# sbelharbi/sr-caco-2

Measured on AMD Instinct MI355X. Metric: train patches/sec, SwinIR x8 64->512 1ch, higher is better.
Workload: dtype f32 (fp16x2 split-MFMA, f32 accumulate)

## Files before the change

include/srhip.h:

```cpp
#ifndef SRHIP_H
#define SRHIP_H
#ifdef __cplusplus
extern "C" {
#endif
#if defined(__GNUC__) || defined(__clang__)
#pragma GCC visibility push(default)
#endif

const char* srhip_last_error(void);
int srhip_abi_version(void);
int srhip_experiments_enabled(void);
int srhip_set_matmul_mode(int mode);
int srhip_get_matmul_mode(void);


int srhip_gemm_nt(const float* A, long lda, const float* W, long ldw, const float* bias, float* C,
                  long ldc, int M, int N, int K, int a_mode, const float* ln_stats, int epi,
                  const float* R, long ldr, const float* rowscale, int rows_per_scale, float alpha,
                  float* aux, long ldaux, void* stream);

int srhip_gemm_nt_batched(const float* A, long lda, long a_z0, long a_z1, const float* W, long ldw, long w_z0, long w_z1, float* C,
                          long ldc, long c_z0, long c_z1, int M, int N, int K, int zcount, int zdiv, void* stream);

int srhip_conv3x3_nhwc(const float* X, long ldx, const float* Wp, const float* bias, float* Y, long ldy,
// ... 134 lines not shown
int srhip_tn_plan_bx3(int M, int NI, int NJ, int conv, int* S, long* part_floats);
int srhip_tn_group_plan_bx3(int M, int ntiles, int* S);
int srhip_gemm_tn_bx3(const float* A, long lda, const float* B, long ldb, int M, int NI, int NJ,
                      const float* a_rowscale, int a_rowscale_rows, int b_mode, const float* ln_stats,
                      float* part, float* part_colsum, int S, void* stream);
int srhip_gemm_tn_grouped_bx3(const srhip_tn_problem* probs, int nprob, int M, int S, void* stream);
int srhip_conv3x3_wgrad_bx3(const float* dY, long lddy, const float* X, long ldx, int B, int H, int W,
                            int Cout, int Cin, float* part, float* part_colsum, int S, void* stream);
int srhip_reduce_linear_wgrad(const float* part, const float* colsum, int S, float* dW, float* db,
                              int N, int K, void* stream);
long srhip_ln_affine_ws(int N, int K);
int srhip_reduce_ln_linear_wgrad(const float* part, const float* colsum, int S, const float* W,
                                 const float* gamma, const float* beta, float* dW, float* db,
                                 float* dgamma, float* dbeta, int N, int K, float* ln_ws,
                                 void* stream);
typedef struct {
  const float* part; const float* colsum;
  const float* W; const float* gamma; const float* beta;
  float* dW; float* db; float* dgamma; float* dbeta;
  int N, K;
  float* ln_ws;
} srhip_reduce_problem;
int srhip_reduce_wgrad_grouped(const srhip_reduce_problem* probs, int nprob, int S, void* stream);
int srhip_reduce_conv_wgrad(const float* part, const float* colsum, int S, float* dW, float* db,
                            int Co, int Ci, void* stream);

int srhip_fold_layernorm(const float* W, const float* b, const float* gamma, const float* beta,
                         float* Wf, float* bf, int N, int K, void* stream);
int srhip_transpose(const float* in, float* out, int R, int C, void* stream);
int srhip_pack_conv_weight(const float* w, float* wp, float* wpt, int Co, int Ci, void* stream);

int srhip_layernorm_fwd(const float* x, float* stats, float* y, const float* gamma, const float* beta,
                        long M, int C, void* stream);
long srhip_layernorm_bwd_ws(long M, int C);
int srhip_layernorm_bwd(const float* dy, const float* x, const float* stats, const float* res,
                        const float* gamma, float* out, float* dgamma, float* dbeta, float* workspace, long M,
                        int C, void* stream);

int srhip_resize_cubic(const void* src, void* dst, int is_u8, int B, int H, int W, int Ho, int Wo, void* stream);
int srhip_u8_to_unit(const unsigned char* src, float* dst, long n, void* stream);
int srhip_clip01(float* x, long n, void* stream);

int srhip_imresize_aa(const void* src, int is_u8, float* tmp, float* dst, int B, int H, int W, int Ho, int Wo, double scale,
                      void* stream);
int srhip_imresize_aa_u16(const unsigned short* src, int in_max, float* tmp, float* dst, int B, int H, int W, int Ho, int Wo,
                          double scale, void* stream);
// ... 293 lines not shown
```

sr-caco-2_amd/csrc/api.hip:

```cpp
#include <stdarg.h>
#include "common.h"
#include "kernels.h"
#include "../../include/srhip.h"

static thread_local char g_err[512] = "";

int sr_fail(int code, const char* fmt, ...) {
  va_list ap;
  va_start(ap, fmt);
  vsnprintf(g_err, sizeof(g_err), fmt, ap);
  va_end(ap);
  return code;
}

extern "C" {

const char* srhip_last_error(void) { return g_err; }
int srhip_abi_version(void) { return 14; }
int srhip_experiments_enabled(void) {
#ifdef SRHIP_EXPERIMENTS
  return 1;
#else
  return 0;
#endif
// ... 423 lines not shown
  SR_REQUIRE(nprob >= 1 && nprob <= (bx ? 24 : 4), "gemm_tn_grouped: 1..%d problems", bx ? 24 : 4);
  SR_REQUIRE(M > 0 && S > 0, "gemm_tn_grouped: empty problem");
  TnArgs a[24];
  memset(a, 0, sizeof(a));
  for (int k = 0; k < nprob; ++k) {
    const srhip_tn_problem& q = probs[k];
    SR_REQUIRE(q.b_mode >= 0 && q.b_mode <= 2, "gemm_tn_grouped: b_mode %d", q.b_mode);
    SR_REQUIRE(q.b_mode != 1 || q.ln_stats, "gemm_tn_grouped: layernorm prologue without stats");
    SR_REQUIRE(!q.a_rowscale || q.a_rowscale_rows > 0, "gemm_tn_grouped: a_rowscale_rows must be > 0");
    TnArgs& p = a[k];
    p.A = q.A; p.lda = q.lda; p.B = q.B; p.ldb = q.ldb; p.M = M; p.NI = q.NI; p.NJ = q.NJ;
    p.a_rowscale = q.a_rowscale; p.a_rowscale_rows = q.a_rowscale_rows; p.b_mode = q.b_mode;
    p.ln_stats = q.ln_stats; p.part = q.part; p.part_colsum = q.part_colsum; p.S = S;
  }
  return bx ? sr_gemm_tnb_grouped(a, nprob, (hipStream_t)stream) : sr_gemm_tn_grouped(a, nprob, (hipStream_t)stream);
}
int srhip_gemm_tn_grouped(const srhip_tn_problem* probs, int nprob, int M, int S, void* stream) {
  return gemm_tn_grouped_any(false, probs, nprob, M, S, stream);
}
int srhip_gemm_tn_grouped_bx3(const srhip_tn_problem* probs, int nprob, int M, int S, void* stream) {
  return gemm_tn_grouped_any(true, probs, nprob, M, S, stream);
}

static int conv3x3_ps2_split(int wfmt, const float* X, long ldx, const void* Wb, const float* bias, float* Yup, long ldy,
                          int B, int H, int W, int Cin, int Cout, int epi, float alpha, void* stream) {
  SR_REQUIRE(epi == 0 || epi == 1 || epi == 6, "conv3x3_ps2_bx3: epi %d (0 bias | 1 relu | 6 leaky relu)", epi);
  NtArgs p;
  memset(&p, 0, sizeof(p));
  p.A = X; p.lda = ldx; p.Wb = (const unsigned short*)Wb; p.C = Yup; p.ldc = ldy;
  p.N = Cout; p.K = Cin; p.bias = bias; p.epi = epi; p.rows_per_scale = H * W; p.alpha = alpha;
  p.batch = B; p.H = H; p.Wd = W; p.ps = 1; p.wfmt = wfmt;
  return sr_conv3x3_ntb(p, (hipStream_t)stream);
}
static int conv3x3_ps2_bwd_data_split(int wfmt, const float* dYup, long lddy, const void* Wbt, float* dX, long ldx, int B, int H,
                                   int W, int Cout, int Cin, int epi, const float* R, long ldr, float alpha,
                                   void* stream) {
  SR_REQUIRE(epi == 0 || ((epi == 4 || epi == 7) && R), "conv3x3_ps2_bwd_data_bx3: epi %d (0 | 4, 7 with R)", epi);
  NtArgs p;
  memset(&p, 0, sizeof(p));
  p.A = dYup; p.lda = lddy; p.Wb = (const unsigned short*)Wbt; p.C = dX; p.ldc = ldx;
  p.N = Cin; p.K = Cout; p.rows_per_scale = H * W; p.alpha = epi == 7 ? alpha : 1.f; p.batch = B; p.H = H; p.Wd = W; p.ps = 2;
  p.epi = epi; p.R = R; p.ldr = ldr; p.wfmt = wfmt;
  return sr_conv3x3_ntb(p, (hipStream_t)stream);
}
int srhip_conv3x3_ps2_bx3(const float* X, long ldx, const void* Wb, const float* bias, float* Yup, long ldy,
                          int B, int H, int W, int Cin, int Cout, int epi, float alpha, void* stream) {
// ... 46 lines not shown
```

sr-caco-2_amd/csrc/gemm_tnb.hip:

```cpp
#include <stdlib.h>
#include "common.h"
#include "kernels.h"

typedef __bf16 bf16x8 __attribute__((ext_vector_type(8)));
typedef __bf16 bf16x2 __attribute__((ext_vector_type(2)));
typedef float f32x2 __attribute__((ext_vector_type(2)));
typedef unsigned u32x4 __attribute__((ext_vector_type(4)));

namespace {

constexpr int TKB = 32;

__device__ const float k_tnb_zero_row[256] = {0.f};

__device__ __forceinline__ f32x16 mfma_bf(u32x4 a, u32x4 b, f32x16 c) {
  return __builtin_amdgcn_mfma_f32_32x32x16_bf16(__builtin_bit_cast(bf16x8, a),
                                                 __builtin_bit_cast(bf16x8, b), c, 0, 0, 0);
}

typedef _Float16 f16x8 __attribute__((ext_vector_type(8)));
typedef _Float16 tn_f16x2 __attribute__((ext_vector_type(2)));
__device__ __forceinline__ f32x16 mfma_h(u32x4 a, u32x4 b, f32x16 c) {
  return __builtin_amdgcn_mfma_f32_32x32x16_f16(__builtin_bit_cast(f16x8, a), __builtin_bit_cast(f16x8, b), c, 0, 0, 0);
}
// ... 307 lines not shown
        const int row = (wi * W + i) * 32 + mfma_row(q, lane);
        if (row < ivalid) {
          const int io = i0 + row;
          out[(long)(p.ps ? (io % ps_f) * 4 + io / ps_f : io) * p.NJ + j0 + col] = acc[i][j][q];
        }
      }
    }
  }

  if (do_colsum) {
    float* red = (float*)smem;
    if (producer && !isB) {
#pragma unroll
      for (int j = 0; j < W; ++j) red[hh * BC + W * lane + j] = cs[j];
    }
    __syncthreads();
    if (tid < ivalid) {
      const int io = i0 + tid;
      p.part_colsum[(long)s * p.NI + (p.ps ? (io % ps_f) * 4 + io / ps_f : io)] = red[tid] + red[BC + tid];
    }
  }
}

template <int W, int BM = -1, bool AR = false, bool NR = false, bool CONV = false>
__device__ __forceinline__ void tnb_body_h(const TnArgs& p, const int s, const int tile, unsigned char* smem, const int tap = 0) {
  const int bmode = BM >= 0 ? BM : p.b_mode;
  const bool arow = BM >= 0 ? AR : (p.a_rowscale != nullptr);
  constexpr int BC = 64 * W, HC = 32 * W;
  constexpr int PLANE = 2 * BC * 64;
  constexpr int BUF = 3 * PLANE;
  constexpr int CTRL = 2 * PLANE;
  constexpr int SINV = 2 * PLANE + 4096;

  const int tid = threadIdx.x, lane = tid & 63;
  const int wave8 = __builtin_amdgcn_readfirstlane(tid >> 6);
  const bool producer = wave8 >= 4;
  const int wave = wave8 & 3;
  const int wi = wave >> 1, wj = wave & 1, r = lane & 31, h = lane >> 5;
  const int nbj = (p.NJ + p.j_tile - 1) / p.j_tile;
  const int bi = tile / nbj, bj = tile - bi * nbj;
  const int i0 = bi * p.i_tile, j0 = bj * p.j_tile;
  const int ivalid = min(p.i_tile, p.NI - i0), jvalid = min(p.j_tile, p.NJ - j0);
  const int m_begin = s * p.rows_per_slice;
  const int m_end = min(p.M, m_begin + p.rows_per_slice);
  const bool do_colsum = p.part_colsum && bj == 0 && tap == 0;
  const int cdy = CONV ? tap / 3 - 1 : 0, cdx = CONV ? tap % 3 - 1 : 0;

  struct Stage {
    typename ColVec<W>::T rv[2][8];
    float scale;
    float2 stats;
    int trow;
  };
  Stage sg0, sg1;
  const bool isB = wave & 1;
  const int ch = wave >> 1;
  const int lt = lane & 31, th = lane >> 5;
  const int opvalid = isB ? jvalid : ivalid;
  const int gcol = HC * ch + W * lt;
  const int colq = max(min(gcol, opvalid - W), 0);
  const int dsh = gcol - colq;
  const bool ragged = NR ? false : opvalid % W != 0;
  const float* const opP = isB ? p.B + j0 : p.A + i0;
  const long opLd = isB ? p.ldb : p.lda;
  const unsigned colb = (unsigned)((16L * th * opLd + colq) * 4);
  float cs[W], sc[W];
#pragma unroll
  for (int j = 0; j < W; ++j) { cs[j] = 0.f; sc[j] = 0x1p126f; }
// ... 256 lines not shown
#pragma unroll
      for (int ks = 0; ks < 2; ++ks) {
        u32x4 fa[W][2];
#pragma unroll
        for (int i = 0; i < W; ++i)
#pragma unroll
          for (int pl = 0; pl < 2; ++pl) fa[i][pl] = *(const u32x4*)(cur + pl * PLANE + a_off[i][ks]);
#pragma unroll
        for (int j = 0; j < W; ++j) {
          const u32x4 bh = *(const u32x4*)(cur + b_off[j][ks]);
          const u32x4 bl = *(const u32x4*)(cur + PLANE + b_off[j][ks]);
#pragma unroll
          for (int i = 0; i < W; ++i) acc[i][j] = mfma_h(fa[i][1], bh, acc[i][j]);
#pragma unroll
          for (int i = 0; i < W; ++i) acc[i][j] = mfma_h(fa[i][0], bl, acc[i][j]);
#pragma unroll
          for (int i = 0; i < W; ++i) acc[i][j] = mfma_h(fa[i][0], bh, acc[i][j]);
        }
      }
      __syncthreads();
    }
    __syncthreads();
    const float* sinv = (const float*)(smem + SINV);
    float* out = p.part + ((long)(s * (CONV ? 9 : 1) + tap) * p.NI) * p.NJ;
#pragma unroll
    for (int i = 0; i < W; ++i)
#pragma unroll
      for (int j = 0; j < W; ++j) {
        const int col = (wj * W + j) * 32 + r;
        if (col >= jvalid) continue;
        const float ib = sinv[BC + col];
#pragma unroll
        for (int q = 0; q < 16; ++q) {
          const int row = (wi * W + i) * 32 + mfma_row(q, lane);
          if (row < ivalid) out[(long)(i0 + row) * p.NJ + j0 + col] = acc[i][j][q] * (sinv[row] * ib);
        }
      }
  }

  if (do_colsum) {
    float* red = (float*)smem;
    if (producer && !isB) {
#pragma unroll
      for (int j = 0; j < W; ++j) red[th * BC + gcol + j] = cs[j];
    }
    __syncthreads();
    if (tid < ivalid) p.part_colsum[(long)s * p.NI + i0 + tid] = red[tid] + red[BC + tid];
  }
}

constexpr int TK9 = 16;
__device__ __forceinline__ int unit_slot9(int col, int u) { return 2 * col + (u ^ ((col >> 3) & 1)); }
constexpr int T9_OPS = 6;
constexpr int T9_PLANE = T9_OPS * 64 * 32;
constexpr int T9_CTRL = 2 * T9_PLANE;
constexpr int T9_BUF = 2 * T9_PLANE + 2048;
constexpr int T9_SINV = 2 * T9_BUF;
constexpr int T9_LDS = 2 * T9_BUF + 2048;
constexpr int T9_THREADS = 14 * 64;

template <int H2, int DBG = 0>
__device__ __forceinline__ void tnb9_consume(const TnArgs& p, const int s, const int i0, const int j0, const int nch,
                                             unsigned char* smem, const int wi, const int wj, const int lane) {
  constexpr int NU = H2 ? 4 : 5;
  constexpr int DY0 = H2 ? 1 : 0;
  const int r = lane & 31, h = lane >> 5;
  f32x16 acc[NU];
#pragma unroll
  for (int u = 0; u < NU; ++u)
#pragma unroll
    for (int q = 0; q < 16; ++q) acc[u][q] = 0.f;
// ... 538 lines not shown
#pragma unroll
  for (int i = 1; i < TNB_GROUP_MAX; ++i)
    if (i < g.n && t >= g.tile_start[i]) { p = g.p[i]; t0 = g.tile_start[i]; }
  tnb_body<W>(p, slice, t - t0, 0, smem);
}

template <int W>
__global__ void __launch_bounds__(512, 1) k_tnb_grouped_h(TnbGroup g) {
  extern __shared__ __attribute__((aligned(16))) unsigned char smem[];
  int slice, t;
  tnb_group_block(g, slice, t);
  TnArgs p = g.p[0];
  int t0 = 0;
#pragma unroll
  for (int i = 1; i < TNB_GROUP_MAX; ++i)
    if (i < g.n && t >= g.tile_start[i]) { p = g.p[i]; t0 = g.tile_start[i]; }
  const bool even = p.NI % W == 0 && p.NJ % W == 0 && p.i_tile % W == 0 && p.j_tile % W == 0;
  if (even && p.b_mode == 1 && !p.a_rowscale) tnb_body_h<W, 1, false, true>(p, slice, t - t0, smem);
  else if (even && p.b_mode == 0 && p.a_rowscale) tnb_body_h<W, 0, true, true>(p, slice, t - t0, smem);
  else if (even && p.b_mode == 2 && p.a_rowscale) tnb_body_h<W, 2, true, true>(p, slice, t - t0, smem);
  else tnb_body_h<W>(p, slice, t - t0, smem);
}

constexpr int TNB_BATCH_MAX = 40;
struct TnbConvBatch {
  TnArgs base;
  const float* A[TNB_BATCH_MAX];
  const float* B[TNB_BATCH_MAX];
  long part_stride, colsum_stride;
  int n, tiles, xcd;
};
template <int W>
__global__ void __launch_bounds__(512, 1) k_tnb_conv_batched(TnbConvBatch g) {
  extern __shared__ __attribute__((aligned(16))) unsigned char smem[];
  const int L = g.xcd ? sr_xcd_block(blockIdx.x, gridDim.x) : (int)blockIdx.x;
  const int tap = L % 9;
  int rr = L / 9;
  const int tile = rr % g.tiles; rr /= g.tiles;
  const int sl = rr % g.base.S, k = rr / g.base.S;
  TnArgs p = g.base;
  p.A = g.A[k];
  p.B = g.B[k];
  p.part = g.base.part + (long)k * g.part_stride;
  p.part_colsum = g.base.part_colsum ? g.base.part_colsum + (long)k * g.colsum_stride : nullptr;
  tnb_body<W>(p, sl, tile, tap, smem);
}
// ... 129 lines not shown
  dim3 grid(probs[0].S * tiles, 1, 1);
  static bool attr[4] = {false, false, false, false};
#define SR_TNB_G(W_)                                                                      \
  if (w == W_) {                                                                          \
    if (!attr[W_]) {                                                                      \
      if (int rc = reserve_lds(k_tnb_grouped<W_>, lds_bytes(W_), "k_tnb_grouped")) return rc; \
      attr[W_] = true;                                                                    \
    }                                                                                     \
    hipLaunchKernelGGL((k_tnb_grouped<W_>), grid, dim3(512), lds_bytes(W_), st, g);       \
  }
  if (w == 3) {
    static bool attr_h = false;
    if (!attr_h) {
      if (int rc = reserve_lds(k_tnb_grouped_h<3>, lds_bytes(3), "k_tnb_grouped_h")) return rc;
      attr_h = true;
    }
    hipLaunchKernelGGL((k_tnb_grouped_h<3>), grid, dim3(512), lds_bytes(3), st, g);
  }
  SR_TNB_G(1) SR_TNB_G(2)
#undef SR_TNB_G
  SR_LAUNCH_CHECK("k_tnb_grouped");
  return 0;
}

int sr_gemm_tnb(TnArgs& p, hipStream_t st) {
  SR_REQUIRE(p.M > 0 && p.S > 0, "gemm_tn_bx3: empty problem");
  SR_REQUIRE(p.NI % 4 == 0 && p.NJ % 4 == 0 && p.lda % 4 == 0 && p.ldb % 4 == 0,
             "gemm_tn_bx3: NI, NJ, lda, ldb must be multiples of 4");
  int tile;
  const int w = pick_w(p.NI, p.NJ, &tile);
  p.i_tile = p.j_tile = tile;
  SR_REQUIRE(!p.ps || (p.conv && p.NI % 4 == 0 && (p.NI / 4) % w == 0 && p.NI % p.i_tile == 0),
             "conv3x3_wgrad + PixelShuffle(2): Cout/4 = %d must be a multiple of %d (columns per lane), Cout of the tile", p.NI / 4, w);
  const int rps = sr_cdiv(p.M, p.S);
  p.rows_per_slice = (rps + TKB - 1) / TKB * TKB;
  int tiles = sr_cdiv(p.NI, p.i_tile) * sr_cdiv(p.NJ, p.j_tile);
  dim3 grid(p.S, tiles, 1);
  if (p.conv) grid = dim3(p.S * tiles * 9, 1, 1);
  static const int xcd = [] { const char* e = sr_getenv("SRHIP_TN_XCD"); return !(e && e[0] == '0'); }();
  const TnbForm form = tnb_form(p);
  if (form == TNB_STRIP9) {
    p.i_tile = p.j_tile = 64;
    tiles = sr_cdiv(p.NI, 64) * sr_cdiv(p.NJ, 64);
    p.aux = p.part + (long)p.S * 9 * p.NI * p.NJ;
    static bool attr9s = false;
    if (!attr9s) {
// ... 164 lines not shown
```

sr-caco-2_amd/csrc/kernels.h:

```cpp
#pragma once
#include <hip/hip_runtime.h>

struct NtArgs {
  const float* A; long lda;
  const float* W; long ldw; long wtap;
  float* C; long ldc;
  int M, N, K;
  int n_tile;
  int xcd_order;
  const float* bias;
  int a_mode;
  const float* ln_stats;
  int epi;
  const float* slope;
  const float* pro_coef;
  const float* R; long ldr;
  float* aux; long ldaux;
  const float* R2; long ldr2; const float* ep_stats;
  int wide_epi;
  float* stats_out;
  const float* rowscale; int rows_per_scale; float alpha;
  int batch, H, Wd, tiles_x, tiles_y;
  int dbg;
  int stagger;
// ... 107 lines not shown
struct PrepEntry {
  const float* a; const float* b; const float* c; void* out; void* out2;
  int kind, blk0;
  int n0, n1, n2;
  int s0, s1, s2, off;
  int mode;
};
int sr_prep_blocks(const PrepEntry& e);
int sr_prep_table(const PrepEntry* tab_dev, int n, int total_blocks, hipStream_t st);
__host__ __device__ static inline int sr_kp(int K) { return (K + 31) / 32 * 32; }
int sr_split3(const float* W, long ldw, int rows, int K, unsigned short* out, hipStream_t st);
int sr_gemm_ntb(NtArgs& p, hipStream_t st);
int sr_conv3x3_ntb(NtArgs& p, hipStream_t st);
int sr_gemm_ntb_lnbwd(NtArgs& p, hipStream_t st);
int sr_gemm_ntp(NtArgs& p, hipStream_t st);
int sr_gemm_ntw(NtArgs& p, hipStream_t st);
int sr_conv3x3_ntcw(NtArgs& p, hipStream_t st);
int sr_conv3x3_ntcw2(NtArgs& p, int rows_per_wave, hipStream_t st);
int sr_conv3x3_nhcw(NtArgs& p, hipStream_t st);
int sr_conv3x3_nhcw2(NtArgs& p, int rows_per_wave, hipStream_t st);
int sr_gemm_tn(TnArgs& p, hipStream_t st);
int sr_gemm_tnb(TnArgs& p, hipStream_t st);
int sr_gemm_tnb_grouped(TnArgs* probs, int n, hipStream_t st);
int sr_tn_plan(int M, int NI, int NJ, int conv, int* S, long* part_floats);
int sr_gemm_tn_grouped(TnArgs* probs, int n, hipStream_t st);
int sr_tn_group_plan(int M, int ntiles, int* S);
int sr_tn_plan_t(int M, int NI, int NJ, int conv, int target, int* S, long* part_floats);
int sr_tn_plan_bx3(int M, int NI, int NJ, int conv, int* S, long* part_floats);
int sr_tn_group_plan_t(int M, int ntiles, int dflt_target, int* S);
int sr_tn_tiles(int NI, int NJ);
int sr_conv_wgrad_batched_plan(int n, int M, int NI, int NJ, int* S, long* part_floats_per_item);
int sr_conv_wgrad_batched_tnb(const TnArgs& base, const float* const* A, const float* const* B, int n,
                              long part_stride, long colsum_stride, hipStream_t st);
```

sr-caco-2_amd/csrc/misc.hip:

```cpp
#include "common.h"
#include "kernels.h"
#include "../../include/srhip.h"

namespace {

__global__ void k_reduce_slices(const float* __restrict__ part, float* __restrict__ out,
                                long n, int S, float beta, const float* __restrict__ colsum,
                                float* __restrict__ db, int nb, int main_blocks) {
  if ((int)blockIdx.x >= main_blocks) {
    const int j = (blockIdx.x - main_blocks) * blockDim.x + threadIdx.x;
    if (j < nb) {
      float d = 0.f;
      for (int s = 0; s < S; ++s) d += colsum[(long)s * nb + j];
      db[j] = d;
    }
    return;
  }
  for (long i = blockIdx.x * (long)blockDim.x + threadIdx.x; i < n;
       i += (long)main_blocks * blockDim.x) {
    float a = 0.f;
    int s = 0;
    for (; s + 8 <= S; s += 8) {
      float v[8];
#pragma unroll
// ... 211 lines not shown
      } else {
        P.dW[(long)n * K + k] = G;
      }
    }
  }
  if (P.gamma) {
    sg[rr][c] = ag; sb[rr][c] = ab;
    __syncthreads();
    if (rr == 0 && k < K) {
      float* w2 = P.lnws + (long)by * 2 * K;
      w2[k] = (sg[0][c] + sg[1][c]) + (sg[2][c] + sg[3][c]);
      w2[K + k] = (sb[0][c] + sb[1][c]) + (sb[2][c] + sb[3][c]);
    }
  }
}
__global__ void __launch_bounds__(256) k_ln_affine_finish_group(ReduceGroup g) {
  ReduceGroup::P P = g.p[0];
  bool found = false;
#pragma unroll
  for (int i = 0; i < 24; ++i)
    if (i < g.n && g.p[i].gamma && (int)blockIdx.x >= g.p[i].fblk0) { P = g.p[i]; found = true; }
  if (!found) return;
  ln_affine_finish_one(P.lnws, (P.N + RG_ROWS - 1) / RG_ROWS, P.K, P.dgamma, P.dbeta, ((int)blockIdx.x - P.fblk0) * 256 + threadIdx.x);
}
__global__ void k_reduce_colsum(const float* __restrict__ colsum, float* __restrict__ db,
                                int N, int S) {
  const int n = blockIdx.x * blockDim.x + threadIdx.x;
  if (n >= N) return;
  float d = 0.f;
  for (int s = 0; s < S; ++s) d += colsum[(long)s * N + n];
  db[n] = d;
}

__global__ void k_fold_ln(const float* __restrict__ W, const float* __restrict__ b,
                          const float* __restrict__ gamma, const float* __restrict__ beta,
                          float* __restrict__ Wf, float* __restrict__ bf, int N, int K) {
  const int n = blockIdx.x * (blockDim.x >> 6) + (threadIdx.x >> 6);
  const int lane = threadIdx.x & 63;
  if (n >= N) return;
  float a = 0.f;
  for (int k = lane; k < K; k += 64) {
    const float w = W[(long)n * K + k];
    Wf[(long)n * K + k] = w * gamma[k];
    a += w * beta[k];
  }
  a = wave_sum(a);
// ... 486 lines not shown
  ReduceGroup g;
  memset(&g, 0, sizeof(g));
  g.n = nprob; g.S = S;
  int blocks = 0, fblocks = 0;
  for (int i = 0; i < nprob; ++i) {
    const srhip_reduce_problem& q = probs[i];
    SR_REQUIRE(q.part && q.colsum && q.dW && q.db && q.N > 0 && q.K > 0, "reduce_wgrad_grouped: problem %d incomplete", i);
    SR_REQUIRE(!q.gamma || (q.W && q.beta && q.dgamma && q.dbeta && q.ln_ws), "reduce_wgrad_grouped: LayerNorm problem %d incomplete", i);
    ReduceGroup::P& d = g.p[i];
    d.lnws = q.ln_ws;
    d.fblk0 = fblocks;
    if (q.gamma) fblocks += sr_cdiv(2 * q.K, 256);
    d.part = q.part; d.colsum = q.colsum; d.W = q.W; d.gamma = q.gamma; d.beta = q.beta;
    d.dW = q.dW; d.db = q.db; d.dgamma = q.dgamma; d.dbeta = q.dbeta; d.N = q.N; d.K = q.K;
    d.blk0 = blocks; d.kblocks = sr_cdiv(q.K, 64);
    blocks += d.kblocks * sr_cdiv(q.N, RG_ROWS);
  }
  hipLaunchKernelGGL(k_reduce_group, dim3(blocks), dim3(256), 0, (hipStream_t)stream, g);
  if (fblocks) hipLaunchKernelGGL(k_ln_affine_finish_group, dim3(fblocks), dim3(256), 0, (hipStream_t)stream, g);
  SR_LAUNCH_CHECK("reduce_wgrad_grouped");
  return 0;
}

int srhip_reduce_conv_wgrad(const float* part, const float* colsum, int S, float* dW, float* db,
                            int Co, int Ci, void* stream) {
  hipStream_t st = (hipStream_t)stream;
  const int mb = ew_grid((long)Co * Ci * 9);
  const bool bias = colsum && db;
  hipLaunchKernelGGL(k_reduce_conv_w, dim3(mb + (bias ? 1 : 0)), dim3(256), 0, st, part, dW, Co, Ci, S,
                     colsum, db, mb);
  SR_LAUNCH_CHECK("reduce_conv_wgrad");
  return 0;
}

int srhip_conv3x3_wgrad_batched_plan(int n, int B, int H, int W, int Cout, int Cin, int* S,
                                     long* part_floats_per_item) {
  SR_REQUIRE(n >= 1 && n <= 40, "conv3x3_wgrad_batched_plan: 1..40 problems (got %d)", n);
  return sr_conv_wgrad_batched_plan(n, B * H * W, Cout, Cin, S, part_floats_per_item);
}

int srhip_conv3x3_wgrad_batched_bx3(const srhip_conv_wgrad_item* items, int n, long lddy, long ldx, int B, int H,
                                    int W, int Cout, int Cin, float* part, float* part_colsum, int S,
                                    void* stream) {
  SR_REQUIRE(n >= 1 && n <= 40, "conv3x3_wgrad_batched: 1..40 problems (got %d)", n);
  SR_REQUIRE(items && part && part_colsum, "conv3x3_wgrad_batched: NULL argument");
  hipStream_t st = (hipStream_t)stream;
// ... 268 lines not shown
```

sr-caco-2_amd/srhip/ops.py:

```python
import ctypes

import torch

from . import probe
from ._lib import call, lib, struct, SrhipError


def _chk(*ts):
    for t in ts:
        if t is None:
            continue
        if not t.is_cuda:
            raise SrhipError("srhip ops need CUDA/HIP tensors (no CPU fallback exists)")
        if t.dtype not in (torch.float32, torch.float64, torch.int32):
            raise SrhipError(f"unsupported dtype {t.dtype}")


def _p(t):
    return None if t is None else t.data_ptr()


def _st():
    return torch.cuda.current_stream().cuda_stream

# ... 1029 lines not shown
    _chk(dY, X, dW, db, a_rowscale, ln_stats)
    M, N = dY.shape
    K = X.shape[1]
    S, n = tn_plan(M, N, K)
    part = SCRATCH.get("tn_part", n, device=dY.device)
    cs = SCRATCH.get("tn_colsum", S * N, device=dY.device)
    call("srhip_gemm_tn" + _tn_sfx(), _p(dY), dY.stride(0), _p(X), X.stride(0), M, N, K, _p(a_rowscale),
         a_rowscale_rows, b_mode, _p(ln_stats), _p(part), _p(cs), S, _st())
    if ln is None:
        call("srhip_reduce_linear_wgrad", _p(part), _p(cs), S, _p(dW), _p(db), N, K, _st())
    else:
        W, gamma, beta, dgamma, dbeta = ln
        lnws = SCRATCH.get("ln_affine_ws", lib.srhip_ln_affine_ws(N, K), device=dY.device)
        call("srhip_reduce_ln_linear_wgrad", _p(part), _p(cs), S, _p(W), _p(gamma), _p(beta),
             _p(dW), _p(db), _p(dgamma), _p(dbeta), N, K, _p(lnws), _st())


_TnProblem = struct("srhip_tn_problem")


_ReduceProblem = struct("srhip_reduce_problem")


def linear_wgrad_grouped(problems):
    n = len(problems)
    M = problems[0]["dY"].shape[0]
    dev = problems[0]["dY"].device
    tiles = sum(lib.srhip_tn_tiles(q["dY"].shape[1], q["X"].shape[1]) for q in problems)
    S = ctypes.c_int(0)
    call("srhip_tn_group_plan" + _tn_sfx(), M, tiles, ctypes.addressof(S))
    S = S.value
    sizes = [(q["dY"].shape[1] * q["X"].shape[1], q["dY"].shape[1]) for q in problems]
    part = SCRATCH.get("tng_part", S * sum(a for a, _ in sizes), device=dev)
    cs = SCRATCH.get("tng_colsum", S * sum(b for _, b in sizes), device=dev)
    arr = (_TnProblem * n)()
    views = []
    po = co = 0
    for k, q in enumerate(problems):
        dY, X = q["dY"], q["X"]
        _chk(dY, X, q["dW"], q["db"], q.get("a_rowscale"), q.get("ln_stats"))
        N, K = dY.shape[1], X.shape[1]
        pk, ck = part[po:po + S * N * K], cs[co:co + S * N]
        po += S * N * K
        co += S * N
        views.append((pk, ck))
        a = arr[k]
        a.A, a.lda, a.B, a.ldb, a.NI, a.NJ = _p(dY), dY.stride(0), _p(X), X.stride(0), N, K
        a.a_rowscale, a.a_rowscale_rows = _p(q.get("a_rowscale")), q.get("a_rowscale_rows", 1)
        a.b_mode, a.ln_stats = q.get("b_mode", 0), _p(q.get("ln_stats"))
        a.part, a.part_colsum = _p(pk), _p(ck)
# ... 1211 lines not shown
```

Baseline: 742.4.

## Balance grouped linear weight-grad GEMM across CUs with even segment planning

Adds a stream-K style host planner that divides the total (tile x K-chunk) work of the grouped weight-gradient GEMMs evenly over a CU-multiple of blocks. Each block handles up to two segments and writes each one to its own partial slot. A matching grouped reduce kernel then sums the slots per tile, and a wider LayerNorm-affine finish kernel is included. The aim is to remove tail imbalance from the fixed split-S scheme. The cost is extra planning tables, a per-shape cached plan, and more partial-slot traffic.

```diff
diff --git a/include/srhip.h b/include/srhip.h
--- a/include/srhip.h
+++ b/include/srhip.h
@@ -180,6 +180,17 @@
   float* ln_ws;
 } srhip_reduce_problem;
 int srhip_reduce_wgrad_grouped(const srhip_reduce_problem* probs, int nprob, int S, void* stream);
+
+typedef struct srhip_tn_even_seg { int tile, m_begin, m_end, slot; } srhip_tn_even_seg;
+typedef struct srhip_tn_even_tile { int first_slot, n_slots; } srhip_tn_even_tile;
+int srhip_tn_even_blocks(int* G);
+int srhip_tn_even_plan_bx3(const int* NI, const int* NJ, int nprob, int M, int G, srhip_tn_even_seg* segs,
+                           srhip_tn_even_tile* tiles_out, int* info);
+int srhip_gemm_tn_grouped_even_bx3(const srhip_tn_problem* probs, int nprob, int M, int G, const srhip_tn_even_seg* segs_dev,
+                                   int slots, float* part, float* colsum, void* stream);
+int srhip_reduce_wgrad_grouped_even(const srhip_reduce_problem* probs, int nprob, int M, int G,
+                                    const srhip_tn_even_tile* tiles_dev, int slots, const float* part, const float* colsum,
+                                    void* stream);
 int srhip_reduce_conv_wgrad(const float* part, const float* colsum, int S, float* dW, float* db,
                             int Co, int Ci, void* stream);
 
diff --git a/sr-caco-2_amd/csrc/api.hip b/sr-caco-2_amd/csrc/api.hip
--- a/sr-caco-2_amd/csrc/api.hip
+++ b/sr-caco-2_amd/csrc/api.hip
@@ -469,6 +469,35 @@
   return gemm_tn_grouped_any(true, probs, nprob, M, S, stream);
 }
 
+int srhip_tn_even_blocks(int* G) {
+  SR_REQUIRE(G, "tn_even_blocks: G required");
+  return sr_tn_even_cus(G);
+}
+int srhip_tn_even_plan_bx3(const int* NI, const int* NJ, int nprob, int M, int G, srhip_tn_even_seg* segs,
+                           srhip_tn_even_tile* tiles_out, int* info) {
+  static_assert(sizeof(srhip_tn_even_seg) == 16 && sizeof(srhip_tn_even_tile) == 8, "table entries are plain ints");
+  return sr_tn_even_plan(NI, NJ, nprob, M, G, (int*)segs, (int*)tiles_out, info);
+}
+int srhip_gemm_tn_grouped_even_bx3(const srhip_tn_problem* probs, int nprob, int M, int G, const srhip_tn_even_seg* segs_dev,
+                                   int slots, float* part, float* colsum, void* stream) {
+  SR_REQUIRE(nprob >= 1 && nprob <= 24, "gemm_tn_grouped_even_bx3: 1..24 problems");
+  SR_REQUIRE(M > 0 && G > 0, "gemm_tn_grouped_even_bx3: empty problem");
+  TnArgs a[24];
+  memset(a, 0, sizeof(a));
+  for (int k = 0; k < nprob; ++k) {
+    const srhip_tn_problem& q = probs[k];
+    SR_REQUIRE(q.A && q.B, "gemm_tn_grouped_even_bx3: problem %d without operands", k);
+    SR_REQUIRE(q.b_mode >= 0 && q.b_mode <= 2, "gemm_tn_grouped_even_bx3: b_mode %d", q.b_mode);
+    SR_REQUIRE(q.b_mode != 1 || q.ln_stats, "gemm_tn_grouped_even_bx3: layernorm prologue without stats");
+    SR_REQUIRE(!q.a_rowscale || q.a_rowscale_rows > 0, "gemm_tn_grouped_even_bx3: a_rowscale_rows must be > 0");
+    TnArgs& p = a[k];
+    p.A = q.A; p.lda = q.lda; p.B = q.B; p.ldb = q.ldb; p.M = M; p.NI = q.NI; p.NJ = q.NJ;
+    p.a_rowscale = q.a_rowscale; p.a_rowscale_rows = q.a_rowscale_rows; p.b_mode = q.b_mode;
+    p.ln_stats = q.ln_stats; p.S = 1;
+  }
+  return sr_gemm_tnb_grouped_even(a, nprob, G, (const int*)segs_dev, slots, part, colsum, (hipStream_t)stream);
+}
+
 static int conv3x3_ps2_split(int wfmt, const float* X, long ldx, const void* Wb, const float* bias, float* Yup, long ldy,
                           int B, int H, int W, int Cin, int Cout, int epi, float alpha, void* stream) {
   SR_REQUIRE(epi == 0 || epi == 1 || epi == 6, "conv3x3_ps2_bx3: epi %d (0 bias | 1 relu | 6 leaky relu)", epi);
diff --git a/sr-caco-2_amd/csrc/gemm_tnb.hip b/sr-caco-2_amd/csrc/gemm_tnb.hip
--- a/sr-caco-2_amd/csrc/gemm_tnb.hip
+++ b/sr-caco-2_amd/csrc/gemm_tnb.hip
@@ -1,4 +1,5 @@
 #include <stdlib.h>
+#include <vector>
 #include "common.h"
 #include "kernels.h"
 
@@ -353,8 +354,9 @@
   }
 }
 
-template <int W, int BM = -1, bool AR = false, bool NR = false, bool CONV = false>
-__device__ __forceinline__ void tnb_body_h(const TnArgs& p, const int s, const int tile, unsigned char* smem, const int tap = 0) {
+template <int W, int BM = -1, bool AR = false, bool NR = false, bool CONV = false, bool SEG = false>
+__device__ __forceinline__ void tnb_body_h(const TnArgs& p, const int m_begin, const int m_end, float* const out, const long ldo,
+                                           float* const cso, const int tile, unsigned char* smem, const int tap = 0) {
   const int bmode = BM >= 0 ? BM : p.b_mode;
   const bool arow = BM >= 0 ? AR : (p.a_rowscale != nullptr);
   constexpr int BC = 64 * W, HC = 32 * W;
@@ -363,7 +365,9 @@
   constexpr int CTRL = 2 * PLANE;
   constexpr int SINV = 2 * PLANE + 4096;
 
-  const int tid = threadIdx.x, lane = tid & 63;
+  int tid_ = threadIdx.x;
+  if constexpr (SEG) asm volatile("" : "+v"(tid_));
+  const int tid = tid_, lane = tid & 63;
   const int wave8 = __builtin_amdgcn_readfirstlane(tid >> 6);
   const bool producer = wave8 >= 4;
   const int wave = wave8 & 3;
@@ -372,9 +376,7 @@
   const int bi = tile / nbj, bj = tile - bi * nbj;
   const int i0 = bi * p.i_tile, j0 = bj * p.j_tile;
   const int ivalid = min(p.i_tile, p.NI - i0), jvalid = min(p.j_tile, p.NJ - j0);
-  const int m_begin = s * p.rows_per_slice;
-  const int m_end = min(p.M, m_begin + p.rows_per_slice);
-  const bool do_colsum = p.part_colsum && bj == 0 && tap == 0;
+  const bool do_colsum = cso && bj == 0 && tap == 0;
   const int cdy = CONV ? tap / 3 - 1 : 0, cdx = CONV ? tap % 3 - 1 : 0;
 
   struct Stage {
@@ -677,7 +679,6 @@
     }
     __syncthreads();
     const float* sinv = (const float*)(smem + SINV);
-    float* out = p.part + ((long)(s * (CONV ? 9 : 1) + tap) * p.NI) * p.NJ;
 #pragma unroll
     for (int i = 0; i < W; ++i)
 #pragma unroll
@@ -688,7 +689,7 @@
 #pragma unroll
         for (int q = 0; q < 16; ++q) {
           const int row = (wi * W + i) * 32 + mfma_row(q, lane);
-          if (row < ivalid) out[(long)(i0 + row) * p.NJ + j0 + col] = acc[i][j][q] * (sinv[row] * ib);
+          if (row < ivalid) out[(long)row * ldo + col] = acc[i][j][q] * (sinv[row] * ib);
         }
       }
   }
@@ -700,8 +701,19 @@
       for (int j = 0; j < W; ++j) red[th * BC + gcol + j] = cs[j];
     }
     __syncthreads();
-    if (tid < ivalid) p.part_colsum[(long)s * p.NI + i0 + tid] = red[tid] + red[BC + tid];
-  }
+    if (tid < ivalid) cso[tid] = red[tid] + red[BC + tid];
+  }
+}
+template <int W, int BM = -1, bool AR = false, bool NR = false, bool CONV = false>
+__device__ __forceinline__ void tnb_body_h(const TnArgs& p, const int s, const int tile, unsigned char* smem, const int tap = 0) {
+  const int nbj = (p.NJ + p.j_tile - 1) / p.j_tile;
+  const int bi = tile / nbj, bj = tile - bi * nbj;
+  const int i0 = bi * p.i_tile, j0 = bj * p.j_tile;
+  const int m_begin = s * p.rows_per_slice;
+  const int m_end = min(p.M, m_begin + p.rows_per_slice);
+  float* out = p.part + ((long)(s * (CONV ? 9 : 1) + tap) * p.NI + i0) * p.NJ + j0;
+  tnb_body_h<W, BM, AR, NR, CONV>(p, m_begin, m_end, out, p.NJ, p.part_colsum ? p.part_colsum + (long)s * p.NI + i0 : nullptr,
+                                  tile, smem, tap);
 }
 
 constexpr int TK9 = 16;
@@ -1286,6 +1298,44 @@
   else tnb_body_h<W>(p, slice, t - t0, smem);
 }
 
+struct TnbEvenGroup {
+  TnArgs p[TNB_GROUP_MAX];
+  int tile_start[TNB_GROUP_MAX + 1];
+  const int4* seg;
+  float* part; float* colsum;
+  long slot_floats;
+  int cs_floats, n, slots;
+};
+template <int W>
+__global__ void __launch_bounds__(512, 1) k_tnb_grouped_even_h(TnbEvenGroup g) {
+  extern __shared__ __attribute__((aligned(16))) unsigned char smem[];
+  const int tiles = g.tile_start[g.n];
+  for (int e = 0; e < 2; ++e) {
+    const int4 sg = g.seg[2 * blockIdx.x + e];
+    const int t = __builtin_amdgcn_readfirstlane(sg.x), m_begin = __builtin_amdgcn_readfirstlane(sg.y);
+    const int m_end = __builtin_amdgcn_readfirstlane(sg.z), slot = __builtin_amdgcn_readfirstlane(sg.w);
+    if (t < 0 || t >= tiles || slot < 0 || slot >= g.slots || m_begin < 0 || m_begin >= m_end || m_end > g.p[0].M ||
+        m_begin % TKB != 0)
+      continue;
+    __syncthreads();
+    int k = 0;
+#pragma unroll
+    for (int i = 1; i < TNB_GROUP_MAX; ++i)
+      if (i < g.n && t >= g.tile_start[i]) k = i;
+    k = __builtin_amdgcn_readfirstlane(k);
+    const TnbEvenGroup* ka = (const TnbEvenGroup*)__builtin_amdgcn_kernarg_segment_ptr();
+    const TnArgs p = ka->p[k];
+    const int t0 = ka->tile_start[k];
+    float* out = g.part + (long)slot * g.slot_floats;
+    float* cso = g.colsum + (long)slot * g.cs_floats;
+    const bool even = p.NI % W == 0 && p.NJ % W == 0 && p.i_tile % W == 0 && p.j_tile % W == 0;
+    if (even && p.b_mode == 1 && !p.a_rowscale) tnb_body_h<W, 1, false, true, false, true>(p, m_begin, m_end, out, p.j_tile, cso, t - t0, smem);
+    else if (even && p.b_mode == 0 && p.a_rowscale) tnb_body_h<W, 0, true, true, false, true>(p, m_begin, m_end, out, p.j_tile, cso, t - t0, smem);
+    else if (even && p.b_mode == 2 && p.a_rowscale) tnb_body_h<W, 2, true, true, false, true>(p, m_begin, m_end, out, p.j_tile, cso, t - t0, smem);
+    else tnb_body_h<W, -1, false, false, false, true>(p, m_begin, m_end, out, p.j_tile, cso, t - t0, smem);
+  }
+}
+
 constexpr int TNB_BATCH_MAX = 40;
 struct TnbConvBatch {
   TnArgs base;
@@ -1461,6 +1511,140 @@
   SR_LAUNCH_CHECK("k_tnb_grouped");
   return 0;
 }
+
+int sr_tn_even_plan(const int* NI, const int* NJ, int n, int M, int G, int* seg, int* tile_tab, int* info) {
+  SR_REQUIRE(n >= 1 && n <= TNB_GROUP_MAX && M > 0 && G > 0 && NI && NJ && info, "tn_even_plan: 1..%d problems, M > 0, G > 0",
+             TNB_GROUP_MAX);
+  long T = 0;
+  int slot_floats = 0, cs_floats = 0, w = 1;
+  long ptiles[TNB_GROUP_MAX];
+  for (int k = 0; k < n; ++k) {
+    SR_REQUIRE(NI[k] > 0 && NJ[k] > 0, "tn_even_plan: problem %d is empty", k);
+    int a, b;
+    const int ti = pick_tile(NI[k], &a), tj = pick_tile(NJ[k], &b);
+    ptiles[k] = (long)sr_cdiv(NI[k], ti) * sr_cdiv(NJ[k], tj);
+    T += ptiles[k];
+    if (ti * tj > slot_floats) slot_floats = ti * tj;
+    if (ti > cs_floats) cs_floats = ti;
+    if (a > w) w = a;
+    if (b > w) w = b;
+  }
+  const long C = sr_cdiv(M, TKB), U = T * C;
+  const long blocks = (long)G * ((T + G - 1) / G);
+  SR_REQUIRE(T < (1 << 20) && blocks < (1 << 24), "tn_even_plan: %ld tiles", T);
+  std::vector<int> order(T);
+  {
+    long g = T, r = blocks % T;
+    while (r) { const long x = g % r; g = r; r = x; }
+    const long P = T / g;
+    if (P <= 1 || P >= T) {
+      for (long q = 0; q < T; ++q) order[q] = (int)q;
+    } else {
+      std::vector<long> used(P, 0), cap(P);
+      for (long c = 0; c < P; ++c) cap[c] = (T - c + P - 1) / P;
+      long tile = 0;
+      for (int k = 0; k < n; ++k) {
+        long c = 0;
+        while (c < P && cap[c] - used[c] < ptiles[k]) ++c;
+        for (long i = 0; i < ptiles[k]; ++i, ++tile) {
+          if (c >= P || used[c] >= cap[c]) {
+            c = 0;
+            for (long x = 1; x < P; ++x)
+              if (cap[x] - used[x] > cap[c] - used[c]) c = x;
+          }
+          order[c + P * used[c]++] = (int)tile;
+        }
+      }
+    }
+  }
+  int slots = 0;
+  if (tile_tab)
+    for (long t = 0; t < T; ++t) tile_tab[2 * t] = tile_tab[2 * t + 1] = 0;
+  for (long b = 0; b < blocks; ++b) {
+    long u = b * U / blocks;
+    const long u1 = (b + 1) * U / blocks;
+    for (int e = 0; e < 2; ++e) {
+      int* q = seg ? seg + (2 * b + e) * 4 : nullptr;
+      if (u >= u1) {
+        if (q) { q[0] = -1; q[1] = q[2] = q[3] = 0; }
+        continue;
+      }
+      const long lp = u / C, c0 = u - lp * C;
+      const long c1 = u1 - lp * C < C ? u1 - lp * C : C;
+      const long t = order[lp];
+      if (q) {
+        q[0] = (int)t; q[1] = (int)(c0 * TKB); q[2] = (int)(c1 * TKB < M ? c1 * TKB : M); q[3] = slots;
+      }
+      if (tile_tab) {
+        if (tile_tab[2 * t + 1] == 0) tile_tab[2 * t] = slots;
+        ++tile_tab[2 * t + 1];
+      }
+      ++slots;
+      u = lp * C + c1;
+    }
+    SR_REQUIRE(u >= u1, "tn_even_plan: a run of more than two segments");
+  }
+  info[0] = (int)blocks; info[1] = (int)T; info[2] = slots; info[3] = slot_floats; info[4] = cs_floats; info[5] = (int)C; info[6] = w;
+  return 0;
+}
+
+int sr_tn_even_cus(int* G) {
+  static int cus = 0;
+  if (!cus) {
+    int dev = 0;
+    hipDeviceProp_t prop;
+    hipError_t e = hipGetDevice(&dev);
+    if (e == hipSuccess) e = hipGetDeviceProperties(&prop, dev);
+    if (e != hipSuccess) return sr_fail(-5, "tn_even_cus: %s", hipGetErrorString(e));
+    cus = prop.multiProcessorCount > 0 ? prop.multiProcessorCount : 1;
+  }
+  *G = cus;
+  return 0;
+}
+
+int sr_gemm_tnb_grouped_even(TnArgs* probs, int n, int G, const int* seg_dev, int slots, float* part, float* colsum,
+                             hipStream_t st) {
+  SR_REQUIRE(n >= 1 && n <= TNB_GROUP_MAX, "gemm_tn_grouped_even_bx3: 1..%d problems (got %d)", TNB_GROUP_MAX, n);
+  SR_REQUIRE(seg_dev && part && colsum && G > 0 && slots > 0, "gemm_tn_grouped_even_bx3: table, part and colsum required");
+  static_assert(sizeof(TnbEvenGroup) <= 4096, "kernel arguments");
+  TnbEvenGroup g;
+  memset(&g, 0, sizeof(g));
+  g.n = n;
+  int tiles = 0;
+  int ni[TNB_GROUP_MAX], nj[TNB_GROUP_MAX];
+  for (int k = 0; k < n; ++k) {
+    TnArgs& p = probs[k];
+    SR_REQUIRE(p.M == probs[0].M && p.M > 0 && !p.conv, "gemm_tn_grouped_even_bx3: problems must share M > 0");
+    SR_REQUIRE(p.NI > 0 && p.NJ > 0 && p.NI % 4 == 0 && p.NJ % 4 == 0 && p.lda % 4 == 0 && p.ldb % 4 == 0,
+               "gemm_tn_grouped_even_bx3: NI, NJ, lda, ldb must be multiples of 4");
+    int a, b;
+    p.i_tile = pick_tile(p.NI, &a);
+    p.j_tile = pick_tile(p.NJ, &b);
+    p.part = nullptr; p.part_colsum = nullptr;
+    g.tile_start[k] = tiles;
+    tiles += sr_cdiv(p.NI, p.i_tile) * sr_cdiv(p.NJ, p.j_tile);
+    g.p[k] = p;
+    ni[k] = p.NI; nj[k] = p.NJ;
+  }
+  g.tile_start[n] = tiles;
+  int info[7];
+  if (int rc = sr_tn_even_plan(ni, nj, n, probs[0].M, G, nullptr, nullptr, info)) return rc;
+  SR_REQUIRE(info[2] == slots, "gemm_tn_grouped_even_bx3: %d slots do not match the plan of this group (%d)", slots, info[2]);
+  const int blocks = info[0];
+  g.seg = (const int4*)seg_dev;
+  g.part = part; g.colsum = colsum;
+  g.slot_floats = info[3]; g.cs_floats = info[4]; g.slots = slots;
+  static bool attr = false;
+  if (!attr) {
+    if (int rc = reserve_lds(k_tnb_grouped_even_h<3>, lds_bytes(3), "k_tnb_grouped_even_h")) return rc;
+    attr = true;
+  }
+  hipLaunchKernelGGL((k_tnb_grouped_even_h<3>), dim3(blocks), dim3(512), lds_bytes(3), st, g);
+  SR_LAUNCH_CHECK("k_tnb_grouped_even_h");
+  return 0;
+}
+
+int sr_tn_pick_tile(int n) { int w; return pick_tile(n, &w); }
 
 int sr_gemm_tnb(TnArgs& p, hipStream_t st) {
   SR_REQUIRE(p.M > 0 && p.S > 0, "gemm_tn_bx3: empty problem");
diff --git a/sr-caco-2_amd/csrc/kernels.h b/sr-caco-2_amd/csrc/kernels.h
--- a/sr-caco-2_amd/csrc/kernels.h
+++ b/sr-caco-2_amd/csrc/kernels.h
@@ -153,6 +153,11 @@
 int sr_gemm_tn(TnArgs& p, hipStream_t st);
 int sr_gemm_tnb(TnArgs& p, hipStream_t st);
 int sr_gemm_tnb_grouped(TnArgs* probs, int n, hipStream_t st);
+int sr_tn_even_plan(const int* NI, const int* NJ, int n, int M, int G, int* seg, int* tile_tab, int* info);
+int sr_tn_even_cus(int* G);
+int sr_gemm_tnb_grouped_even(TnArgs* probs, int n, int G, const int* seg_dev, int slots, float* part, float* colsum,
+                             hipStream_t st);
+int sr_tn_pick_tile(int n);
 int sr_tn_plan(int M, int NI, int NJ, int conv, int* S, long* part_floats);
 int sr_gemm_tn_grouped(TnArgs* probs, int n, hipStream_t st);
 int sr_tn_group_plan(int M, int ntiles, int* S);
diff --git a/sr-caco-2_amd/csrc/misc.hip b/sr-caco-2_amd/csrc/misc.hip
--- a/sr-caco-2_amd/csrc/misc.hip
+++ b/sr-caco-2_amd/csrc/misc.hip
@@ -257,6 +257,128 @@
     if (i < g.n && g.p[i].gamma && (int)blockIdx.x >= g.p[i].fblk0) { P = g.p[i]; found = true; }
   if (!found) return;
   ln_affine_finish_one(P.lnws, (P.N + RG_ROWS - 1) / RG_ROWS, P.K, P.dgamma, P.dbeta, ((int)blockIdx.x - P.fblk0) * 256 + threadIdx.x);
+}
+struct ReduceEvenGroup {
+  struct P {
+    const float* W; const float* gamma; const float* beta;
+    float* dW; float* db; float* lnws;
+    int N, K, blk0, kblocks, tile0, it, jt;
+  } p[24];
+  const float* part; const float* colsum; const int2* tiles;
+  long slot_floats;
+  int cs_floats, n, slots;
+};
+__global__ void __launch_bounds__(256) k_reduce_group_even(ReduceEvenGroup g) {
+  __shared__ float sd[RG_ROWS], sg[4][64], sb[4][64];
+  ReduceEvenGroup::P P = g.p[0];
+#pragma unroll
+  for (int i = 1; i < 24; ++i)
+    if (i < g.n && (int)blockIdx.x >= g.p[i].blk0) P = g.p[i];
+  const int N = P.N, K = P.K;
+  const int lb = blockIdx.x - P.blk0;
+  const int bx = lb % P.kblocks, by = lb / P.kblocks;
+  const int c = threadIdx.x & 63, rr = threadIdx.x >> 6;
+  const int k = bx * 64 + c;
+  const int nbj = (K + P.jt - 1) / P.jt;
+  auto slots_of = [&](int tile, int& first) -> int {
+    const int2 ts = g.tiles[P.tile0 + tile];
+    first = max(ts.x, 0);
+    return max(min(ts.y, g.slots - first), 0);
+  };
+  if (threadIdx.x < RG_ROWS) {
+    const int n = by * RG_ROWS + threadIdx.x;
+    float d = 0.f;
+    if (n < N) {
+      const int bi = n / P.it;
+      int first;
+      const int cnt = slots_of(bi * nbj, first);
+      const float* q = g.colsum + (long)first * g.cs_floats + (n - bi * P.it);
+      for (int s = 0; s < cnt; ++s) d += q[(long)s * g.cs_floats];
+    }
+    sd[threadIdx.x] = d;
+    if (n < N && bx == 0) P.db[n] = d;
+  }
+  __syncthreads();
+  float ag = 0.f, ab = 0.f;
+  const long sl = g.slot_floats;
+  const float gk = (P.gamma && k < K) ? P.gamma[k] : 0.f, bk = (P.gamma && k < K) ? P.beta[k] : 0.f;
+  const int bj = k < K ? k / P.jt : 0;
+#pragma unroll
+  for (int pass = 0; pass < RG_ROWS / 4; ++pass) {
+    const int n = by * RG_ROWS + pass * 4 + rr;
+    if (k < K && n < N) {
+      const int bi = n / P.it;
+      int first;
+      const int S = slots_of(bi * nbj + bj, first);
+      const float* pp = g.part + first * sl + (long)(n - bi * P.it) * P.jt + (k - bj * P.jt);
+      float G = 0.f;
+      int s = 0;
+      for (; s + 8 <= S; s += 8) {
+        float v[8];
+#pragma unroll
+        for (int u = 0; u < 8; ++u) v[u] = pp[(s + u) * sl];
+#pragma unroll
+        for (int u = 0; u < 8; ++u) G += v[u];
+      }
+      for (; s + 4 <= S; s += 4) {
+        float v[4];
+#pragma unroll
+        for (int u = 0; u < 4; ++u) v[u] = pp[(s + u) * sl];
+#pragma unroll
+        for (int u = 0; u < 4; ++u) G += v[u];
+      }
+      for (; s < S; ++s) G += pp[s * sl];
+      if (P.gamma) {
+        const float d = sd[pass * 4 + rr];
+        const float w = P.W[(long)n * K + k];
+        P.dW[(long)n * K + k] = gk * G + bk * d;
+        ag += w * G;
+        ab += w * d;
+      } else {
+        P.dW[(long)n * K + k] = G;
+      }
+    }
+  }
+  if (P.gamma) {
+    sg[rr][c] = ag; sb[rr][c] = ab;
+    __syncthreads();
+    if (rr == 0 && k < K) {
+      float* w2 = P.lnws + (long)by * 2 * K;
+      w2[k] = (sg[0][c] + sg[1][c]) + (sg[2][c] + sg[3][c]);
+      w2[K + k] = (sb[0][c] + sb[1][c]) + (sb[2][c] + sb[3][c]);
+    }
+  }
+}
+__global__ void __launch_bounds__(1024) k_ln_affine_finish_group_wide(ReduceGroup g) {
+  __shared__ float sm[16][64];
+  ReduceGroup::P P = g.p[0];
+  bool found = false;
+#pragma unroll
+  for (int i = 0; i < 24; ++i)
+    if (i < g.n && g.p[i].gamma && (int)blockIdx.x >= g.p[i].fblk0) { P = g.p[i]; found = true; }
+  if (!found) return;
+  const int K = P.K, nrb = (P.N + RG_ROWS - 1) / RG_ROWS;
+  const int c = threadIdx.x & 63, rl = threadIdx.x >> 6;
+  const int idx = ((int)blockIdx.x - P.fblk0) * 64 + c;
+  const int which = idx >= K, k = idx - which * K;
+  float a0 = 0.f, a1 = 0.f, a2 = 0.f, a3 = 0.f;
+  if (idx < 2 * K) {
+    const float* q = P.lnws + (long)which * K + k;
+    int rb = rl;
+    for (; rb + 48 < nrb; rb += 64) {
+      a0 += q[(long)(rb + 0) * 2 * K]; a1 += q[(long)(rb + 16) * 2 * K];
+      a2 += q[(long)(rb + 32) * 2 * K]; a3 += q[(long)(rb + 48) * 2 * K];
+    }
+    for (; rb < nrb; rb += 16) a0 += q[(long)rb * 2 * K];
+  }
+  sm[rl][c] = (a0 + a1) + (a2 + a3);
+  __syncthreads();
+  if (rl == 0 && idx < 2 * K) {
+    float t = 0.f;
+#pragma unroll
+    for (int r = 0; r < 16; ++r) t += sm[r][c];
+    (which ? P.dbeta : P.dgamma)[k] = t;
+  }
 }
 __global__ void k_reduce_colsum(const float* __restrict__ colsum, float* __restrict__ db,
                                 int N, int S) {
@@ -789,6 +911,48 @@
   return 0;
 }
 
+int srhip_reduce_wgrad_grouped_even(const srhip_reduce_problem* probs, int nprob, int M, int G,
+                                    const srhip_tn_even_tile* tiles_dev, int slots, const float* part, const float* colsum,
+                                    void* stream) {
+  SR_REQUIRE(nprob >= 1 && nprob <= 24 && slots > 0, "reduce_wgrad_grouped_even: 1..24 problems, slots > 0");
+  SR_REQUIRE(tiles_dev && part && colsum, "reduce_wgrad_grouped_even: table, part and colsum required");
+  ReduceEvenGroup g;
+  ReduceGroup f;
+  memset(&g, 0, sizeof(g));
+  memset(&f, 0, sizeof(f));
+  g.n = f.n = nprob;
+  int blocks = 0, fblocks = 0, tiles = 0;
+  int ni[24], nj[24];
+  for (int i = 0; i < nprob; ++i) {
+    const srhip_reduce_problem& q = probs[i];
+    SR_REQUIRE(q.dW && q.db && q.N > 0 && q.K > 0, "reduce_wgrad_grouped_even: problem %d incomplete", i);
+    SR_REQUIRE(!q.gamma || (q.W && q.beta && q.dgamma && q.dbeta && q.ln_ws), "reduce_wgrad_grouped_even: LayerNorm problem %d incomplete", i);
+    ReduceEvenGroup::P& d = g.p[i];
+    d.W = q.W; d.gamma = q.gamma; d.beta = q.beta; d.dW = q.dW; d.db = q.db; d.lnws = q.ln_ws;
+    d.N = q.N; d.K = q.K;
+    d.it = sr_tn_pick_tile(q.N); d.jt = sr_tn_pick_tile(q.K);
+    d.tile0 = tiles;
+    tiles += sr_cdiv(q.N, d.it) * sr_cdiv(q.K, d.jt);
+    d.blk0 = blocks; d.kblocks = sr_cdiv(q.K, 64);
+    blocks += d.kblocks * sr_cdiv(q.N, RG_ROWS);
+    ReduceGroup::P& e = f.p[i];
+    e.gamma = q.gamma; e.lnws = q.ln_ws; e.dgamma = q.dgamma; e.dbeta = q.dbeta; e.N = q.N; e.K = q.K;
+    e.fblk0 = fblocks;
+    if (q.gamma) fblocks += sr_cdiv(2 * q.K, 64);
+    ni[i] = q.N; nj[i] = q.K;
+  }
+  int info[7];
+  if (int rc = sr_tn_even_plan(ni, nj, nprob, M, G, nullptr, nullptr, info)) return rc;
+  SR_REQUIRE(info[1] == tiles && info[2] == slots, "reduce_wgrad_grouped_even: %d slots do not match the plan of this group (%d)",
+             slots, info[2]);
+  g.part = part; g.colsum = colsum; g.tiles = (const int2*)tiles_dev;
+  g.slot_floats = info[3]; g.cs_floats = info[4]; g.slots = slots;
+  hipLaunchKernelGGL(k_reduce_group_even, dim3(blocks), dim3(256), 0, (hipStream_t)stream, g);
+  if (fblocks) hipLaunchKernelGGL(k_ln_affine_finish_group_wide, dim3(fblocks), dim3(1024), 0, (hipStream_t)stream, f);
+  SR_LAUNCH_CHECK("reduce_wgrad_grouped_even");
+  return 0;
+}
+
 int srhip_reduce_conv_wgrad(const float* part, const float* colsum, int S, float* dW, float* db,
                             int Co, int Ci, void* stream) {
   hipStream_t st = (hipStream_t)stream;
diff --git a/sr-caco-2_amd/srhip/ops.py b/sr-caco-2_amd/srhip/ops.py
--- a/sr-caco-2_amd/srhip/ops.py
+++ b/sr-caco-2_amd/srhip/ops.py
@@ -1075,10 +1075,101 @@
 _ReduceProblem = struct("srhip_reduce_problem")
 
 
+_TnEvenSeg = struct("srhip_tn_even_seg")
+_TnEvenTile = struct("srhip_tn_even_tile")
+_EVEN_PLANS = {}
+_EVEN_G = {}
+
+
+def wgrad_even():
+    return _os.environ.get("SRHIP_WGRAD_EVEN", "1") != "0"
+
+
+def tn_even_blocks(dev):
+    key = (dev.type, dev.index)
+    if key not in _EVEN_G:
+        G = ctypes.c_int(0)
+        with torch.cuda.device(dev):
+            call("srhip_tn_even_blocks", ctypes.addressof(G))
+        _EVEN_G[key] = G.value
+    return _EVEN_G[key]
+
+
+def tn_even_plan_host(shapes, M, G):
+    n = len(shapes)
+    ni = (ctypes.c_int * n)(*[s[0] for s in shapes])
+    nj = (ctypes.c_int * n)(*[s[1] for s in shapes])
+    info = (ctypes.c_int * 7)()
+    call("srhip_tn_even_plan_bx3", ctypes.addressof(ni), ctypes.addressof(nj), n, M, G, None, None, ctypes.addressof(info))
+    segs = (_TnEvenSeg * (2 * info[0]))()
+    tiles = (_TnEvenTile * info[1])()
+    call("srhip_tn_even_plan_bx3", ctypes.addressof(ni), ctypes.addressof(nj), n, M, G, ctypes.addressof(segs),
+         ctypes.addressof(tiles), ctypes.addressof(info))
+    names = ("blocks", "tiles", "slots", "slot_floats", "colsum_floats", "chunks", "tile_class")
+    return dict(zip(names, info)), segs, tiles
+
+
+def tn_even_plan(shapes, M, dev):
+    key = (dev.type, dev.index, tuple(shapes), M)
+    plan = _EVEN_PLANS.get(key)
+    if plan is None:
+        G = tn_even_blocks(dev)
+        info, segs, tiles = tn_even_plan_host(shapes, M, G)
+        segs_d = torch.frombuffer(bytearray(bytes(segs)), dtype=torch.int32).to(dev)
+        tiles_d = torch.frombuffer(bytearray(bytes(tiles)), dtype=torch.int32).to(dev)
+        plan = _EVEN_PLANS[key] = (info, segs_d, tiles_d, G)
+    return plan
+
+
+def _linear_wgrad_grouped_even(problems):
+    n = len(problems)
+    M = problems[0]["dY"].shape[0]
+    dev = problems[0]["dY"].device
+    shapes = [(q["dY"].shape[1], q["X"].shape[1]) for q in problems]
+    info, segs_d, tiles_d, G = tn_even_plan(shapes, M, dev)
+    slots = info["slots"]
+    part = SCRATCH.get("tng_part", slots * info["slot_floats"], device=dev)
+    cs = SCRATCH.get("tng_colsum", slots * info["colsum_floats"], device=dev)
+    arr = (_TnProblem * n)()
+    for a, q in zip(arr, problems):
+        dY, X = q["dY"], q["X"]
+        _chk(dY, X, q["dW"], q["db"], q.get("a_rowscale"), q.get("ln_stats"))
+        a.A, a.lda, a.B, a.ldb, a.NI, a.NJ = _p(dY), dY.stride(0), _p(X), X.stride(0), dY.shape[1], X.shape[1]
+        a.a_rowscale, a.a_rowscale_rows = _p(q.get("a_rowscale")), q.get("a_rowscale_rows", 1)
+        a.b_mode, a.ln_stats = q.get("b_mode", 0), _p(q.get("ln_stats"))
+
+    def launch():
+        call("srhip_gemm_tn_grouped_even_bx3", ctypes.addressof(arr), n, M, G, _p(segs_d), slots, _p(part), _p(cs), _st())
+    if probe.on("linear_tn"):
+        fl = sum(2.0 * M * a * b for a, b in shapes)
+        by = sum(4.0 * (M * (a + b) + a * b) for a, b in shapes)
+        with probe.timed(("linear_tn", M, n), fl, by):
+            launch()
+    else:
+        launch()
+    red = (_ReduceProblem * n)()
+    lnsz = [lib.srhip_ln_affine_ws(a, b) if q.get("ln") is not None else 0 for q, (a, b) in zip(problems, shapes)]
+    lnws = SCRATCH.get("ln_affine_ws_g", max(1, sum(lnsz)), device=dev)
+    lo = 0
+    for r, q, (N, K), lsz in zip(red, problems, shapes, lnsz):
+        r.dW, r.db, r.N, r.K = _p(q["dW"]), _p(q["db"]), N, K
+        if q.get("ln") is not None:
+            W, gamma, beta, dgamma, dbeta = q["ln"]
+            r.W, r.gamma, r.beta, r.dgamma, r.dbeta = _p(W), _p(gamma), _p(beta), _p(dgamma), _p(dbeta)
+            r.ln_ws = _p(lnws[lo:lo + lsz])
+            lo += lsz
+    call("srhip_reduce_wgrad_grouped_even", ctypes.addressof(red), n, M, G, _p(tiles_d), slots, _p(part), _p(cs), _st())
+
+
 def linear_wgrad_grouped(problems):
     n = len(problems)
     M = problems[0]["dY"].shape[0]
     dev = problems[0]["dY"].device
+    if (wgrad_even() and use_bx3() and F16X2 and lib.srhip_get_matmul_mode() == 0 and 1 <= n <= 24 and M > 0
+            and all(min(q["dY"].shape[1], q["X"].shape[1]) > 0 for q in problems)):
+        shapes = [(q["dY"].shape[1], q["X"].shape[1]) for q in problems]
+        if tn_even_plan(shapes, M, dev)[0]["tile_class"] == 3:
+            return _linear_wgrad_grouped_even(problems)
     tiles = sum(lib.srhip_tn_tiles(q["dY"].shape[1], q["X"].shape[1]) for q in problems)
     S = ctypes.c_int(0)
     call("srhip_tn_group_plan" + _tn_sfx(), M, tiles, ctypes.addressof(S))
```

Result: no change. 746.4, median of 6 (+0.5%).
